# CGLemon/Sayuri

Measured on AMD Instinct MI355X. Metric: nn_evals_per_sec, higher is better.
Workload: dtype f16

## Files before the change

### include/sayuri_hip.h

```cpp
#ifndef SAYURI_HIP_H
#define SAYURI_HIP_H

#include <stddef.h>
#include <stdint.h>

#ifdef __cplusplus
extern "C" {
#endif

typedef struct sayuri_hip_ctx sayuri_hip_ctx;

enum {
    SAYURI_ACT_IDENTITY = 0, SAYURI_ACT_RELU = 1, SAYURI_ACT_ELU = 2, SAYURI_ACT_SELU = 3,
    SAYURI_ACT_GELU = 4, SAYURI_ACT_MISH = 5, SAYURI_ACT_SWISH = 6, SAYURI_ACT_HARDSWISH = 7
};

enum {
    SAYURI_BLOCK_RESIDUAL = 1, SAYURI_BLOCK_BOTTLENECK = 2, SAYURI_BLOCK_NESTED_BOTTLENECK = 3,
    SAYURI_BLOCK_MIXER = 4
};

typedef struct {
    int32_t type;
    int32_t apply_se;
// ... 39 lines not shown
sayuri_hip_ctx* sayuri_hip_create(int device, const sayuri_hip_netdesc* desc, int max_batch,
                                  int board, int use_fp16);

enum { SAYURI_HIP_LATENCY = 1 };
sayuri_hip_ctx* sayuri_hip_create_ex(int device, const sayuri_hip_netdesc* desc, int max_batch,
                                     int board, int use_fp16, unsigned flags);

int sayuri_hip_load_tensor(sayuri_hip_ctx* ctx, int layer_id, int kind, const float* host, size_t n);

int sayuri_hip_forward(sayuri_hip_ctx* ctx, int n, const float* planes, const int* board_sizes,
                       float* prob, float* pass, float* misc, float* own);

int sayuri_hip_upload(sayuri_hip_ctx* ctx, int n, const float* planes, const int* board_sizes);
int sayuri_hip_run(sayuri_hip_ctx* ctx);
int sayuri_hip_sync(sayuri_hip_ctx* ctx);
int sayuri_hip_download(sayuri_hip_ctx* ctx, float* prob, float* pass, float* misc, float* own);

int sayuri_hip_submit(sayuri_hip_ctx* ctx, int n, const float* planes, const int* board_sizes, float* prob,
                      float* pass, float* misc, float* own, int* ticket);
int sayuri_hip_forward_packed(sayuri_hip_ctx* ctx, int n, const unsigned* records, int binary_planes, const int* board_sizes,
                              float* prob, float* pass, float* misc, float* own);
int sayuri_hip_submit_packed(sayuri_hip_ctx* ctx, int n, const unsigned* records, int binary_planes, const int* board_sizes,
                             float* prob, float* pass, float* misc, float* own, int* ticket);
int sayuri_hip_wait(sayuri_hip_ctx* ctx, int ticket);
int sayuri_hip_query(sayuri_hip_ctx* ctx, int ticket);

int sayuri_hip_time_runs(sayuri_hip_ctx* ctx, int iters, float* total_ms);

typedef struct {
    char name[48];
    int32_t launches;
    float total_ms;
    double flops;
    double bytes;
} sayuri_hip_kernel_stat;
int sayuri_hip_profile_run(sayuri_hip_ctx* ctx, sayuri_hip_kernel_stat* rows, int cap);

int sayuri_hip_mark_kernel(sayuri_hip_ctx* ctx, const char* name);
int sayuri_hip_timed_stat(sayuri_hip_ctx* ctx, sayuri_hip_kernel_stat* row);

void* sayuri_hip_host_alloc(size_t bytes);
void sayuri_hip_host_free(void* p);

size_t sayuri_hip_device_bytes(const sayuri_hip_ctx* ctx);

int sayuri_hip_last_chains(const sayuri_hip_ctx* ctx);

int sayuri_hip_tower_state(const sayuri_hip_ctx* ctx);

int sayuri_hip_latency_state(const sayuri_hip_ctx* ctx);

void sayuri_hip_destroy(sayuri_hip_ctx* ctx);

const char* sayuri_hip_last_error(void);

int sayuri_hip_test_conv(int device, int use_fp16, int n, const int* board_sizes, int max_board,
                         int cin, int cout, int k, int depthwise, int act, int post_residual,
                         const float* x, const float* w, const float* bias, const float* res,
                         float* y);
int sayuri_hip_test_conv_split(int device, int n, const int* board_sizes, int max_board, int cin, int cout, int act,
                               const float* x, const float* w, const float* bias, const float* res, float* y,
                               int channel_tiles, int strips);
int sayuri_hip_test_last_conv_kind(void);
int sayuri_hip_test_se_unit(int device, int use_fp16, int n, const int* board_sizes, int max_board, int channels,
                            int se_size, int act, const float* x, const float* res, const float* w1, const float* b1,
                            const float* w2, const float* b2, float* y, float* gate);
int sayuri_hip_test_head_tail(int device, int use_fp16, int n, const int* board_sizes, int max_board, int policy_channels,
                              int value_channels, int prob_channels, int pass_outs, int misc_outs, int act,
                              const float* pconv, const float* vconv, const float* const* weights12, float* prob,
                              float* pass, float* misc, float* own);

int sayuri_hip_test_conv_se(int device, int n, const int* board_sizes, int max_board, int channels, int se_size, int act,
                            int via_tower, const float* x, const float* w, const float* bias, const float* res, const float* w1,
                            const float* b1, const float* w2, const float* b2, float* y);
int sayuri_hip_test_conv_sx(int device, int n, const int* board_sizes, int max_board, int channels, int se_size, int act,
                            const float* x, const float* w, const float* bias, const float* res, const float* w1,
                            const float* b1, const float* w2, const float* b2, float* y);
int sayuri_hip_test_last_sx_kts(void);
int sayuri_hip_test_head_board(int device, int n, const int* board_sizes, int max_board, int channels, int policy_channels,
                               int value_channels, int prob_channels, int pass_outs, int misc_outs, int act, const float* trunk,
                               const float* p_w, const float* p_b, const float* v_w, const float* v_b,
                               const float* const* weights12, float* prob, float* pass, float* misc, float* own);

#ifdef __cplusplus
}
#endif
#endif
```

### sayuri_amd/_lib.py

```python
from __future__ import annotations

import ctypes
import os

from . import _build

c_float_p = ctypes.POINTER(ctypes.c_float)
c_int_p = ctypes.POINTER(ctypes.c_int)


class KernelStat(ctypes.Structure):
    _fields_ = [("name", ctypes.c_char * 48), ("launches", ctypes.c_int32), ("total_ms", ctypes.c_float),
                ("flops", ctypes.c_double), ("bytes", ctypes.c_double)]


HIP_SYMBOLS = [
    "sayuri_hip_device_count", "sayuri_hip_create", "sayuri_hip_create_ex", "sayuri_hip_latency_state", "sayuri_hip_test_conv_split", "sayuri_hip_load_tensor", "sayuri_hip_forward",
    "sayuri_hip_submit", "sayuri_hip_wait", "sayuri_hip_query", "sayuri_hip_upload", "sayuri_hip_run", "sayuri_hip_sync", "sayuri_hip_download", "sayuri_hip_time_runs",
    "sayuri_hip_forward_packed", "sayuri_hip_submit_packed", "sayuri_hip_profile_run", "sayuri_hip_mark_kernel", "sayuri_hip_timed_stat", "sayuri_hip_host_alloc", "sayuri_hip_host_free", "sayuri_hip_device_bytes", "sayuri_hip_last_chains", "sayuri_hip_tower_state",
    "sayuri_hip_destroy", "sayuri_hip_last_error", "sayuri_hip_test_conv", "sayuri_hip_test_last_conv_kind",
    "sayuri_hip_test_se_unit", "sayuri_hip_test_head_tail", "sayuri_hip_test_conv_se", "sayuri_hip_test_head_board",
    "sayuri_hip_test_conv_sx", "sayuri_hip_test_last_sx_kts",
]

_hip = None
_host = None


def _require(path: str) -> str:
    if not os.path.exists(path):
        raise RuntimeError(
            f"native library {path} is missing: run `python -c 'import __graft_entry__ as g; g.build()'` "
            "(there is no CPU fallback for the MI355X forward pipe)")
    return path


def hip() -> ctypes.CDLL:
    global _hip
    if _hip is None:
        path = _build.HIP_SO
        fake = os.environ.get("SAYURI_FAKE_HIP_LIB")
        if fake:
            import sys
            print(f"[sayuri_amd] SAYURI_FAKE_HIP_LIB is set: the device side is the test stand-in {fake}, NOT the MI355X engine",
                  file=sys.stderr)
            path = fake
        lib = ctypes.CDLL(_require(path), mode=ctypes.RTLD_GLOBAL)
        lib.sayuri_hip_last_error.restype = ctypes.c_char_p
        lib.sayuri_hip_device_count.restype = ctypes.c_int
        lib.sayuri_hip_upload.argtypes = [ctypes.c_void_p, ctypes.c_int, c_float_p, c_int_p]
        lib.sayuri_hip_run.argtypes = [ctypes.c_void_p]
        lib.sayuri_hip_sync.argtypes = [ctypes.c_void_p]
        lib.sayuri_hip_download.argtypes = [ctypes.c_void_p, c_float_p, c_float_p, c_float_p, c_float_p]
        lib.sayuri_hip_forward.argtypes = [ctypes.c_void_p, ctypes.c_int, c_float_p, c_int_p, c_float_p,
                                           c_float_p, c_float_p, c_float_p]
        lib.sayuri_hip_time_runs.argtypes = [ctypes.c_void_p, ctypes.c_int, c_float_p]
        lib.sayuri_hip_profile_run.argtypes = [ctypes.c_void_p, ctypes.POINTER(KernelStat), ctypes.c_int]
        lib.sayuri_hip_mark_kernel.argtypes = [ctypes.c_void_p, ctypes.c_char_p]
        lib.sayuri_hip_timed_stat.argtypes = [ctypes.c_void_p, ctypes.POINTER(KernelStat)]
        lib.sayuri_hip_device_bytes.restype = ctypes.c_size_t
        lib.sayuri_hip_device_bytes.argtypes = [ctypes.c_void_p]
        lib.sayuri_hip_last_chains.restype = ctypes.c_int
        lib.sayuri_hip_last_chains.argtypes = [ctypes.c_void_p]
        lib.sayuri_hip_tower_state.restype = ctypes.c_int
        lib.sayuri_hip_tower_state.argtypes = [ctypes.c_void_p]
        if hasattr(lib, "sayuri_hip_latency_state"):
            lib.sayuri_hip_latency_state.restype = ctypes.c_int
            lib.sayuri_hip_latency_state.argtypes = [ctypes.c_void_p]
        if hasattr(lib, "sayuri_hip_create_ex"):
            lib.sayuri_hip_create_ex.restype = ctypes.c_void_p
            lib.sayuri_hip_create_ex.argtypes = [ctypes.c_int, ctypes.c_void_p, ctypes.c_int, ctypes.c_int, ctypes.c_int, ctypes.c_uint]
        if hasattr(lib, "sayuri_hip_test_conv_split"):
            lib.sayuri_hip_test_conv_split.argtypes = [ctypes.c_int, ctypes.c_int, c_int_p, ctypes.c_int, ctypes.c_int, ctypes.c_int,
                                                       ctypes.c_int, c_float_p, c_float_p, c_float_p, c_float_p, c_float_p,
                                                       ctypes.c_int, ctypes.c_int]
        if not fake:
            lib.sayuri_hip_test_conv.argtypes = [ctypes.c_int, ctypes.c_int, ctypes.c_int, c_int_p, ctypes.c_int,
                                                 ctypes.c_int, ctypes.c_int, ctypes.c_int, ctypes.c_int, ctypes.c_int,
                                                 ctypes.c_int, c_float_p, c_float_p, c_float_p, c_float_p, c_float_p]
        _hip = lib
    return _hip


def host() -> ctypes.CDLL:
    global _host
    if _host is None:
        hip()
        lib = ctypes.CDLL(_require(_build.HOST_SO))
        lib.sayuri_host_last_error.restype = ctypes.c_char_p
        lib.sayuri_weights_load.restype = ctypes.c_void_p
        lib.sayuri_weights_load.argtypes = [ctypes.c_char_p]
        lib.sayuri_weights_free.argtypes = [ctypes.c_void_p]
        lib.sayuri_weights_info.argtypes = [ctypes.c_void_p, c_int_p]
        lib.sayuri_weights_block_info.argtypes = [ctypes.c_void_p, ctypes.c_int, c_int_p]
        lib.sayuri_weights_tensor.restype = ctypes.c_long
        lib.sayuri_weights_tensor.argtypes = [ctypes.c_void_p, ctypes.c_char_p, c_float_p, ctypes.c_long]
        lib.sayuri_pipe_create.restype = ctypes.c_void_p
        lib.sayuri_pipe_create.argtypes = [ctypes.c_char_p, ctypes.c_int, ctypes.c_int, ctypes.c_int, ctypes.c_int,
                                           ctypes.c_int]
        lib.sayuri_pipe_create_ex.restype = ctypes.c_void_p
        lib.sayuri_pipe_create_ex.argtypes = [ctypes.c_char_p, ctypes.c_int, ctypes.c_int, ctypes.c_int, ctypes.c_int,
                                              ctypes.c_int, ctypes.c_uint]
        lib.sayuri_pipe_destroy.argtypes = [ctypes.c_void_p]
        lib.sayuri_pipe_num_workers.argtypes = [ctypes.c_void_p]
        lib.sayuri_pipe_ctx.restype = ctypes.c_void_p
# ... 12 lines not shown
```

### sayuri_amd/csrc/hip/engine_graph.h

```cpp
#pragma once
#include "engine_plan.h"

namespace sayuri {

class EngineBase {
public:
    virtual ~EngineBase() {}
    virtual int load_tensor(int layer, int kind, const float* host, size_t n) = 0;
    virtual int upload(int n, const float* planes, const int* board_sizes, const unsigned* packed = nullptr, int binary = 0) = 0;
    virtual int run() = 0;
    virtual int sync() = 0;
    virtual int download(float* prob, float* pass, float* misc, float* own) = 0;
    virtual int time_runs(int iters, float* ms) = 0;
    virtual int profile_run(sayuri_hip_kernel_stat* rows, int cap) = 0;
    virtual int submit(int n, const float* planes, const int* bsz, float* prob, float* pass, float* misc, float* own,
                       int* ticket, const unsigned* packed = nullptr, int binary = 0) = 0;
    virtual int wait(int ticket) = 0;
    virtual int query(int ticket) = 0;
    virtual int mark_kernel(const char* name) = 0;
    virtual int timed_stat(sayuri_hip_kernel_stat* row) = 0;
    virtual size_t device_bytes() const = 0;
    virtual int last_chains() const = 0;
    virtual int tower_state() const = 0;
    virtual int latency_state() const = 0;
// ... 1082 lines not shown
    void rows_reset() {
        for (int i = 0; i < kNumBufs; ++i) rows_stride_[i] = 0;
    }
    int rows_use(const Fwd& f, const ConvParams& p, const char* layer) {
        const void* use[3] = {p.in, p.out, p.res};
        for (int u = 0; u < 3 && flags_.dbg_recycle_input < 2; ++u)
            for (int i = 0; i < kNumBufs; ++i) {
                if (!use[u] || f.io.bufs[i] != use[u]) continue;
                const int stride = u ? p.cout_s : p.cin_s;
                if (rows_stride_[i] && rows_stride_[i] != stride)
                    return fail(std::string("activation buffer ") + std::to_string(i) + " is used with row stride " + std::to_string(stride) + " by " +
                                layer + " and with " + std::to_string(rows_stride_[i]) + " by " + (rows_first_[i] ? rows_first_[i] : "?") +
                                " inside one persistent run / chained forward: the rows of different tiles would overlap");
                rows_stride_[i] = stride;
                rows_first_[i] = layer;
            }
        return 0;
    }

    const ConvLayerDev& cv(int id) const { return convs_.at(id); }
    const FcLayerDev& fc(int id) const { return fcs_.at(id); }

    int forward(int t, float* zc_pass = nullptr, float* zc_misc = nullptr) {
        const int G = chains_for_batch();
        last_chains_ = G;
        rows_reset();
        IoSlot& io = io_[t];
        Fwd f{t, io, compute_[t]};
        f.ntiles = plan().ntiles;
        f.ns = geom_.n;
        f.px = geom_.total;
        f.pass = zc_pass ? zc_pass : io.pass;
        f.misc = zc_misc ? zc_misc : io.misc;
        if (sx_kts_) {
            int nse = 0;
            for (const auto& b : blocks_) nse += b.apply_se ? 1 : 0;
            if (io.sx_epoch > 0xfff00000u) {
                HIP_OK(hipMemsetAsync(io.sx_xchg, 0, sizeof(unsigned long long) * (size_t)max_batch_ * sx_kts_ * kSxMaxSub * kSxSlots, f.stream));
                io.sx_epoch = 0;
            }
            f.sx_epoch0 = io.sx_epoch;
            io.sx_epoch += (unsigned)nse;
        }
        if (G <= 1) return forward_graph(f);
        if (chain_setup(G)) return -1;
        const BoardTabs* tabs = nullptr;
        if (board_tabs(f, &tabs)) return -1;
        HIP_OK(hipEventRecord(chain_fork_, f.stream));
        const int nt = board_plan_.ntiles;
        for (int g = 0; g < G; ++g) {
            Fwd c = f;
            c.stream = chain_stream_[g];
            c.chained = true;
            c.tile0 = (int)((long)nt * g / G);
            c.ntiles = (int)((long)nt * (g + 1) / G) - c.tile0;
            c.n0 = board_plan_.tile_first[c.tile0];
            c.ns = board_plan_.tile_first[c.tile0 + c.ntiles] - c.n0;
            c.px = geom_.off[c.n0 + c.ns] - geom_.off[c.n0];
            hipError_t e = hipStreamWaitEvent(c.stream, chain_fork_, 0);
            if (flags_.chains_serial && g > 0 && e == hipSuccess) e = hipStreamWaitEvent(c.stream, chain_join_[g - 1], 0);
            if (e == hipSuccess && forward_graph(c)) return -1;
            if (e == hipSuccess) e = hipEventRecord(chain_join_[g], c.stream);
            if (e != hipSuccess) return fail(std::string("chained forward: ") + hipGetErrorString(e));
        }
        for (int g = 0; g < G; ++g) HIP_OK(hipStreamWaitEvent(f.stream, chain_join_[g], 0));
        return 0;
    }

    int pack_input(Fwd& f, T* dst) {
        const int cin = desc_.input_channels, cs = cv(SAYURI_L_INPUT_CONV).cin_s, board = board_;
        const int n0 = f.n0, ns = f.ns;
        const double px = f.px;
        const BatchGeom g = dgeom(f.io);
        const IoSlot& io = f.io;
        if (io.packed_binary > 0) {
            const unsigned* rec = io.packed_src ? io.packed_src : io.packed;
            const int split = io.packed_src ? 1 : kPackSplit;
            const int nbin = io.packed_binary, words = nbin * 12 + 8;
            return timed(f, "pack_input", 0, (double)ns * words * 4 + px * cs * sizeof(T), [&] {
                hipLaunchKernelGGL(pack_bits_kernel<T>, dim3(ns * split), dim3(256), 0, f.stream, rec, words, nbin, dst, g, cin, cs,
                                   io.g_perm, n0, split);
            });
        }
        const int grid = ns * kPackSplit;
        const int chunk = pack_input_chunk(slot_pix_, cs, (int)sizeof(T));
        const size_t lds = (size_t)chunk * (cs * sizeof(T) + 16);
        const size_t flat_lds = pack_input_flat_lds(slot_pix_, cs, (int)sizeof(T));
        const bool flat = flat_lds <= 64 * 1024 && (size_t)cin * board * board < 65536;
        return timed(f, "pack_input", 0, px * cin * 4 + px * cs * sizeof(T), [&] {
            if (flat)
                hipLaunchKernelGGL(pack_input_flat_kernel<T>, dim3(ns), dim3(kPackFlatThreads), flat_lds, f.stream,
                                   (const float*)io.planes, dst, g, cin, cs, board, io.g_perm, n0);
            else
                hipLaunchKernelGGL(pack_input_kernel<T>, dim3(grid), dim3(kPackThreads), lds, f.stream,
                                   (const float*)io.planes, dst, g, cin, cs, board, io.g_perm, chunk, n0);
        });
    }

    int forward_graph(Fwd& f) {
        const auto& d = desc_;
        const int C = d.residual_channels, csC = round_up(C, 32), act = d.default_act;
        T* const* buf = f.io.bufs;

        int x = f.take();
        const int in = f.take();
        if (pack_input(f, buf[in])) return -1;
        if (conv(f, "conv3x3_input", cv(SAYURI_L_INPUT_CONV), buf[in], buf[x], nullptr, act)) return -1;
        if (flags_.dbg_recycle_input) f.give(in);

        for (int b = 0; b < d.residual_blocks; ++b) {
            const auto& bd = blocks_[b];
            const bool se = bd.apply_se != 0;
            const int last_act = se ? (int)kIdentity : act;
            const int y = f.take();
            int skip = x;
            bool se_done = false;
            if (bd.type == SAYURI_BLOCK_RESIDUAL) {
                const int t0 = f.take();
                if (conv(f, "conv3x3_tower", cv(SAYURI_L_BLOCK(b, SAYURI_S_CONV1)), buf[x], buf[t0], nullptr, act)) return -1;
                int fused = 1;
                if (se) {
                    fused = conv_se(f, cv(SAYURI_L_BLOCK(b, SAYURI_S_CONV2)), fc(SAYURI_L_BLOCK(b, SAYURI_S_SQUEEZE)),
                                    fc(SAYURI_L_BLOCK(b, SAYURI_S_EXCITE)), buf[t0], buf[y], buf[x], C, act);
                    if (fused == 1)
                        fused = conv_sx(f, cv(SAYURI_L_BLOCK(b, SAYURI_S_CONV2)), fc(SAYURI_L_BLOCK(b, SAYURI_S_SQUEEZE)),
                                        fc(SAYURI_L_BLOCK(b, SAYURI_S_EXCITE)), buf[t0], buf[y], buf[x], C, act);
                    if (fused < 0) return -1;
                    se_done = fused == 0;
                }
                if (fused == 1 &&
                    conv(f, "conv3x3_tower", cv(SAYURI_L_BLOCK(b, SAYURI_S_CONV2)), buf[t0], buf[y], se ? nullptr : buf[x], last_act))
                    return -1;
                f.give(t0);
            } else if (bd.type == SAYURI_BLOCK_BOTTLENECK) {
                const int t0 = f.take(), t1 = f.take();
                if (conv(f, "conv1x1_tower", cv(SAYURI_L_BLOCK(b, SAYURI_S_PRE_BTL)), buf[x], buf[t0], nullptr, act)) return -1;
                if (conv(f, "conv3x3_tower", cv(SAYURI_L_BLOCK(b, SAYURI_S_CONV1)), buf[t0], buf[t1], nullptr, act)) return -1;
                if (conv(f, "conv3x3_tower", cv(SAYURI_L_BLOCK(b, SAYURI_S_CONV2)), buf[t1], buf[t0], nullptr, act)) return -1;
                if (conv(f, "conv1x1_tower", cv(SAYURI_L_BLOCK(b, SAYURI_S_POST_BTL)), buf[t0], buf[y], se ? nullptr : buf[x], last_act)) return -1;
                f.give(t0); f.give(t1);
            } else if (bd.type == SAYURI_BLOCK_NESTED_BOTTLENECK) {
                const int r1 = f.take(), t0 = f.take(), t1 = f.take();
                if (conv(f, "conv1x1_tower", cv(SAYURI_L_BLOCK(b, SAYURI_S_PRE_BTL)), buf[x], buf[r1], nullptr, act)) return -1;
                if (conv(f, "conv3x3_tower", cv(SAYURI_L_BLOCK(b, SAYURI_S_CONV1)), buf[r1], buf[t0], nullptr, act)) return -1;
                if (conv(f, "conv3x3_tower", cv(SAYURI_L_BLOCK(b, SAYURI_S_CONV2)), buf[t0], buf[t1], buf[r1], act)) return -1;
                if (conv(f, "conv3x3_tower", cv(SAYURI_L_BLOCK(b, SAYURI_S_CONV3)), buf[t1], buf[t0], nullptr, act)) return -1;
                if (conv(f, "conv3x3_tower", cv(SAYURI_L_BLOCK(b, SAYURI_S_CONV4)), buf[t0], buf[r1], buf[t1], act)) return -1;
                if (conv(f, "conv1x1_tower", cv(SAYURI_L_BLOCK(b, SAYURI_S_POST_BTL)), buf[r1], buf[y], se ? nullptr : buf[x], last_act)) return -1;
                f.give(r1); f.give(t0); f.give(t1);
            } else {
                const int s2 = f.take(), t1 = f.take();
                if (depthwise(f, "depthwise", cv(SAYURI_L_BLOCK(b, SAYURI_S_DW_CONV)), buf[x], buf[s2], buf[x], act)) return -1;
                if (conv(f, "conv1x1_tower", cv(SAYURI_L_BLOCK(b, SAYURI_S_CONV1)), buf[s2], buf[t1], nullptr, act)) return -1;
                if (conv(f, "conv1x1_tower", cv(SAYURI_L_BLOCK(b, SAYURI_S_CONV2)), buf[t1], buf[y], se ? nullptr : buf[s2], last_act)) return -1;
                f.give(t1);
                f.give(x);
                x = s2;
                skip = s2;
            }
            if (se && !se_done) {
                if (se_unit(f, fc(SAYURI_L_BLOCK(b, SAYURI_S_SQUEEZE)), fc(SAYURI_L_BLOCK(b, SAYURI_S_EXCITE)), buf[y], buf[skip], C, csC,
                            act, f.n0, f.ns))
                    return -1;
            }
            f.give(x);
            x = y;
        }
        return heads(f, x);
    }

    int heads(Fwd& f, int x) {
        const auto& d = desc_;
        const int C = d.residual_channels, csC = round_up(C, 32), act = d.default_act;
        const int Cp = d.policy_head_channels, Cv = d.value_head_channels;
        T* const* buf = f.io.bufs;
        const BatchGeom g = dgeom(f.io);
        const ConvLayerDev &pw = cv(SAYURI_L_PROB_CONV), &ow = cv(SAYURI_L_V_OWNERSHIP);
        const HeadWeights hw{fc(SAYURI_L_P_INTER_FC).dev(), fc(SAYURI_L_PASS_FC).dev(), fc(SAYURI_L_V_INTER_FC).dev(), fc(SAYURI_L_V_MISC).dev(),
                             pw.w32, pw.bias, ow.w32, ow.bias};
// ... 194 lines not shown
```

### sayuri_amd/csrc/hip/engine_plan.h

```cpp
#pragma once
namespace sayuri {

static thread_local std::string g_err;
static std::atomic<unsigned> g_host_free_gen{0};
static thread_local int g_test_conv_kind = 0;
static int fail(const std::string& m) { g_err = m; return -1; }

#define HIP_OK(expr)                                                                      \
    do {                                                                                  \
        hipError_t e_ = (expr);                                                           \
        if (e_ != hipSuccess) {                                                           \
            g_err = std::string(#expr) + ": " + hipGetErrorString(e_);                    \
            return -1;                                                                    \
        }                                                                                 \
    } while (0)

static inline int round_up(int v, int m) { return (v + m - 1) / m * m; }
constexpr size_t kMaxLds = 160 * 1024;
constexpr int kNumCU = 256;

template <typename T> struct ConvKernelTable {
    typedef void (*Fn)(const ConvParams);
    struct Entry { int wmt, wnt; Fn fn; size_t (*lds)(int); int npos_cap; };
    static std::vector<Entry>& entries() {
// ... 487 lines not shown
    img2->assign((size_t)kts * w2_bytes, 0);
    for (int kt = 0; kt < kts; ++kt) {
        for (int bs = 2; bs <= board; ++bs) {
            const float sc = ((float)bs - 14.f) / 10.f;
            f16* d = img1->data() + ((size_t)kt * (board - 1) + (bs - 2)) * (w1_bytes / 2);
            for (int r = 0; r < 256; ++r) {
                const int c = kt * 128 + (r & 127);
                if (c >= C) continue;
                for (int o = 0; o < se; ++o) {
                    const float* w = sq_w + (size_t)o * 3 * C;
                    d[(size_t)r * se + o] = (f16)(r < 128 ? w[c] + sc * w[C + c] : w[2 * C + c]);
                }
            }
        }
        unsigned char* base = img2->data() + (size_t)kt * w2_bytes;
        f16* h = (f16*)base;
        float* bias = (float*)(base + (size_t)se * 256 * 2);
        for (int o = 0; o < 256; ++o) {
            const int c = kt * 128 + (o & 127);
            if (c >= C) continue;
            const int row = o < 128 ? c : C + c;
            for (int i = 0; i < se; ++i) h[((size_t)(i >> 2) * 256 + o) * 4 + (i & 3)] = (f16)ex_w[(size_t)row * se + i];
            bias[o] = ex_b[row];
        }
        std::copy(sq_b, sq_b + se, bias + 256);
    }
    *w1_bytes_out = w1_bytes;
    *w2_bytes_out = w2_bytes;
    return true;
}

struct HeadImages {
    std::vector<f16> img, img2;
    std::vector<float> bias;
    int PT = 0, VT = 0;
};
static HeadFn make_head_images(int C, int Cp, int Cv, int prob_ch, int board, const float* p_w, const float* p_b, const float* v_w,
                               const float* v_b, const float* prob_w, const float* own_w, HeadImages* out) {
    if (board * board > kHeadPix || prob_ch > 8) return nullptr;
    const int PT = round_up(Cp, 16), rows = round_up(PT + Cv, 32), VT = rows - PT, cs = round_up(C, 32), nch = cs / 32;
    HeadFn fn = nullptr;
    for (const auto& e : kHeadEntries)
        if (e.rt * 16 == rows && head_board_fits(rows, nch, e.depth)) { fn = e.fn; break; }
    if (!fn) return nullptr;
    out->img2.assign((size_t)(rows / 32) * 4 * 16 * 8, (f16)0.f);
    for (int t = 0; t < rows / 32; ++t)
        for (int kg = 0; kg < 4; ++kg)
            for (int e = 0; e < 8; ++e) {
                const int ch = 32 * t + (e < 4 ? 4 * kg + e : 16 + 4 * kg + (e - 4));
                for (int k = 0; k < prob_ch; ++k)
                    if (ch < Cp) out->img2[(((size_t)t * 4 + kg) * 16 + k) * 8 + e] = (f16)prob_w[(size_t)k * Cp + ch];
                if (ch >= PT && ch - PT < Cv) out->img2[(((size_t)t * 4 + kg) * 16 + prob_ch) * 8 + e] = (f16)own_w[ch - PT];
            }
    out->img.assign((size_t)nch * 4 * rows * 8, (f16)0.f);
    out->bias.assign(rows, 0.f);
    for (int half = 0; half < 2; ++half) {
        const float* w = half ? v_w : p_w;
        const float* b = half ? v_b : p_b;
        const int cout = half ? Cv : Cp, r0 = half ? PT : 0;
        for (int ko = 0; ko < cout; ++ko) {
            out->bias[r0 + ko] = b[ko];
            for (int c = 0; c < C; ++c)
                out->img[(((size_t)(c / 32) * 4 + (c % 32) / 8) * rows + r0 + ko) * 8 + c % 8] = (f16)w[(size_t)ko * C + c];
        }
    }
    out->PT = PT;
    out->VT = VT;
    return fn;
}

struct HeadWeights {
    FcDev p_inter, pass_fc, v_inter, v_misc;
    const float *prob_w, *prob_b, *own_w, *own_b;
};
static HeadParams head_params(const HeadWeights& w, int Cp, int Cv, int prob_ch, int act, int board, float* prob, float* pass, float* misc,
                              float* own, const int* perm) {
    HeadParams h{};
    h.p_inter = w.p_inter; h.pass_fc = w.pass_fc; h.v_inter = w.v_inter; h.v_misc = w.v_misc;
    h.prob_w = w.prob_w; h.prob_b = w.prob_b; h.own_w = w.own_w; h.own_b = w.own_b;
    h.Cp = Cp; h.cs_p = round_up(Cp, 32); h.Cv = Cv; h.cs_v = round_up(Cv, 32); h.prob_ch = prob_ch; h.act = act; h.board = board;
    h.prob = prob; h.pass = pass; h.misc = misc; h.own = own; h.perm = perm;
    return h;
}
template <typename T, typename Run>
static int se_unit_launches(hipStream_t s, const BatchGeom& g, double px, T* x, const T* res, float* separt, float* gate, const FcDev& sq,
                            const FcDev& ex, int C, int cs, int act, int n0, int ns, Run&& run) {
    constexpr int EPP = ElemTraits<T>::kPieceElems;
    if (cs / EPP > 256) return fail("SE unit: more than 256*8 channels is not supported");
    const double fc = (double)sq.in * sq.out + (double)ex.in * ex.out;
    if (run("se_pool", 2.0 * px * C, sizeof(T) * px * C,
            [&] { hipLaunchKernelGGL(se_pool_kernel<T>, dim3(ns * kSeSplit), dim3(256), 0, s, (const T*)x, separt, g, cs, n0); }))
        return -1;
    const size_t smem = sizeof(float) * (3 * C + sq.out + kSeFcThreads);
    if (run("se_fc", 2.0 * ns * fc, 4.0 * ns * fc, [&] {
            hipLaunchKernelGGL(se_fc_kernel, dim3(ns), dim3(kSeFcThreads), smem, s, (const float*)separt, gate, g, C, cs, sq, ex, act, n0);
        }))
        return -1;
    const dim3 grid((g.slot_pix * (cs / EPP) + 256 * kScaleUnroll - 1) / (256 * kScaleUnroll), ns);
    return run("se_scale", 3.0 * px * C, sizeof(T) * px * C * 3,
               [&] { hipLaunchKernelGGL(se_scale_kernel<T>, grid, dim3(256), 0, s, (const T*)x, res, x, (const float*)gate, g, C, cs, act, n0); });
}

}
extern "C" const unsigned char sayuri_tower_hsaco[];
extern "C" const unsigned long long sayuri_tower_hsaco_size;
namespace sayuri {
static int load_tower_module(hipModule_t* mod, hipFunction_t fn[2]) {
    if (sayuri_tower_hsaco_size == 0) return fail("this build carries no persistent tower kernel: tower_seam.py rejected the compiler's assembly at build time");
    HIP_OK(hipModuleLoadData(mod, sayuri_tower_hsaco));
    HIP_OK(hipModuleGetFunction(&fn[0], *mod, "_ZN6sayuri17conv_tower_kernelILi4EEEvPKNS_10TowerLayerE"));
    HIP_OK(hipModuleGetFunction(&fn[1], *mod, "_ZN6sayuri17conv_tower_kernelILi2EEEvPKNS_10TowerLayerE"));
    return 0;
}

}
```

### sayuri_amd/csrc/hip/engine_taps.h

```cpp
#pragma once
#include "engine_graph.h"

namespace sayuri {

struct TestGeom {
    HostGeom hg;
    int slot = 0;
    int* d_off = nullptr;
    int* d_bsz = nullptr;
    BatchGeom g{};
};

class TestArena {
public:
    ~TestArena() { for (void* p : ptrs_) (void)hipFree(p); }
    void* alloc(size_t bytes) {
        void* p = nullptr;
        if (hipMalloc(&p, std::max<size_t>(bytes, 256)) != hipSuccess) return nullptr;
        (void)hipMemset(p, 0, std::max<size_t>(bytes, 256));
        ptrs_.push_back(p);
        return p;
    }
    template <typename U> U* upload(const std::vector<U>& h) {
        U* d = (U*)alloc(h.size() * sizeof(U));
// ... 339 lines not shown
                             const float* b2, float* y) {
    typedef f16 T;
    constexpr unsigned kEpoch = 0x5e17u;
    g_test_sx_kts = 0;
    HIP_OK(hipSetDevice(device));
    enable_big_lds_glds();
    TestArena A;
    TestGeom tg;
    if (make_test_geom(A, n, board_sizes, max_board, &tg)) return -1;
    const int cs = round_up(C, 32), kts = round_up(C, 128) / 128;
    int wmt, ko_pad;
    conv_tile(cs, true, &wmt, &ko_pad);
    if (cs != kts * 128 || ko_pad != kts * 128) return 1;
    std::vector<f16> img1;
    std::vector<unsigned char> img2;
    int w1_bytes = 0, w2_bytes = 0;
    if (!make_sx_images(C, se, kts, max_board, w1, b1, w2, b2, &img1, &img2, &w1_bytes, &w2_bytes)) return 1;
    const BoardPlan plan = board_plan(tg.hg, ConvOverride{});
    const BoardEntry* be = plan.ok ? sx_board_entry(plan.npos) : nullptr;
    if (!be) return 1;
    for (int i = 0; i < n; ++i)
        if (!sx_board_fused(tg.hg.bsz[i])) return 1;
    const T* dx = A.upload_prefixed(nchw_to_nhwc<T>(tg, x, C, cs));
    const T* dres = res ? A.upload(nchw_to_nhwc<T>(tg, res, C, cs)) : nullptr;
    T* dy = (T*)A.alloc((size_t)n * tg.slot * cs * sizeof(T));
    const T* dw = A.upload(conv_image<T>(w, C, C, 9, ko_pad));
    const float* db = A.upload(padded_bias(bias, C, ko_pad));
    const f16* d1 = A.upload(img1);
    const unsigned char* d2 = A.upload(img2);
    unsigned long long* xchg = (unsigned long long*)A.alloc(sizeof(unsigned long long) * (size_t)plan.ntiles * kts * kSxMaxSub * kSxSlots);
    TestBoardTabs tabs;
    TestHostWord err;
    if (!dx || (res && !dres) || !dy || !dw || !db || !d1 || !d2 || !xchg || !make_board_tabs(A, tg, plan, &tabs) || !err.alloc())
        return fail("test_conv_sx: hipMalloc failed");
    BoardSxParams sp;
    std::memset(&sp, 0, sizeof(sp));
    board_params(sp.b, plan, tabs.src, tabs.pix, tabs.cols, true);
    conv_params(sp.b.c, dx, dw, db, dres, dy, tg.g, cs, cs, ko_pad, 9, act);
    sp.b.c.npos = 0; sp.b.c.num_pix_tiles = plan.ntiles;
    sx_params(sp, d1, d2, w1_bytes, w2_bytes, max_board, se, kts, xchg, kEpoch, err.dev, false);
    HIP_OK(hipMemset(dy, 0xff, (size_t)n * tg.slot * cs * sizeof(T)));
    g_test_conv_kind = kConvBoardSx;
    g_test_sx_kts = kts;
    hipLaunchKernelGGL(conv_board_sx_kernel<2>, dim3(sx_grid(plan.ntiles, kts)), dim3(512), be->lds(plan.npos), 0, sp);
    HIP_OK(hipGetLastError());
    HIP_OK(hipDeviceSynchronize());
    if (*(volatile unsigned*)err.host) return fail("test_conv_sx: a workgroup's wait for its sibling channel tiles ran out");
    return nhwc_to_nchw(tg, dy, C, cs, y);
}

static int test_head_board_impl(int device, int n, const int* board_sizes, int max_board, int C, int Cp, int Cv, int prob_ch,
                                int pass_outs, int misc_outs, int act, const float* trunk, const float* p_w, const float* p_b,
                                const float* v_w, const float* v_b, const float* const* w, float* prob, float* pass, float* misc,
                                float* own) {
    typedef f16 T;
    HIP_OK(hipSetDevice(device));
    enable_big_lds_glds();
    TestArena A;
    TestGeom tg;
    if (make_test_geom(A, n, board_sizes, max_board, &tg)) return -1;
    HeadImages hi;
    const HeadFn fn = make_head_images(C, Cp, Cv, prob_ch, max_board, p_w, p_b, v_w, v_b, w[8], w[10], &hi);
    if (!fn) return 1;
    const int cs = round_up(C, 32);
    const T* dt = A.upload(nchw_to_nhwc<T>(tg, trunk, C, cs));
    const f16* d_img = A.upload(hi.img);
    const f16* d_img2 = A.upload(hi.img2);
    const float* d_bias = A.upload(hi.bias);
    HeadWeights hw;
    TestHeadOut o;
    if (!dt || !d_img || !d_img2 || !d_bias || !upload_head_weights(A, w, Cp, Cv, prob_ch, pass_outs, misc_outs, &hw) ||
        !o.alloc(A, n, prob_ch, pass_outs, misc_outs, max_board * max_board))
        return fail("test_head_board: hipMalloc failed");
    HeadBoardParams hp;
    std::memset(&hp, 0, sizeof(hp));
    hp.h = head_params(hw, Cp, Cv, prob_ch, act, max_board, o.prob, o.pass, o.misc, o.own, nullptr);
    hp.trunk = dt; hp.w = d_img; hp.w2 = d_img2; hp.bias = d_bias; hp.g = tg.g; hp.cs = cs; hp.PT = hi.PT; hp.VT = hi.VT;
    hipLaunchKernelGGL(fn, dim3(n), dim3(512), kMaxLds, 0, hp);
    HIP_OK(hipGetLastError());
    HIP_OK(hipDeviceSynchronize());
    return o.download(prob, pass, misc, own);
}

}

extern "C" int sayuri_hip_test_conv_se(int device, int n, const int* board_sizes, int max_board, int channels, int se_size, int act,
                                       int via_tower, const float* x, const float* w, const float* bias, const float* res,
                                       const float* w1, const float* b1, const float* w2, const float* b2, float* y) {
    if (!board_sizes || !x || !w || !w1 || !b1 || !w2 || !b2 || !y || n <= 0) return fail("test_conv_se: bad argument");
    return test_conv_se_impl(device, n, board_sizes, max_board, channels, se_size, act, via_tower, x, w, bias, res, w1, b1, w2, b2, y);
}

extern "C" int sayuri_hip_test_conv_sx(int device, int n, const int* board_sizes, int max_board, int channels, int se_size, int act,
                                       const float* x, const float* w, const float* bias, const float* res, const float* w1,
                                       const float* b1, const float* w2, const float* b2, float* y) {
    if (!board_sizes || !x || !w || !w1 || !b1 || !w2 || !b2 || !y || n <= 0) return fail("test_conv_sx: bad argument");
    return test_conv_sx_impl(device, n, board_sizes, max_board, channels, se_size, act, x, w, bias, res, w1, b1, w2, b2, y);
}

extern "C" int sayuri_hip_test_last_sx_kts(void) { return sayuri::g_test_sx_kts; }

extern "C" int sayuri_hip_test_head_board(int device, int n, const int* board_sizes, int max_board, int channels, int policy_channels,
                                          int value_channels, int prob_channels, int pass_outs, int misc_outs, int act, const float* trunk,
                                          const float* p_w, const float* p_b, const float* v_w, const float* v_b,
                                          const float* const* weights12, float* prob, float* pass, float* misc, float* own) {
    if (!board_sizes || !trunk || !p_w || !p_b || !v_w || !v_b || !weights12 || !prob || !pass || !misc || !own || n <= 0)
        return fail("test_head_board: bad argument");
    return test_head_board_impl(device, n, board_sizes, max_board, channels, policy_channels, value_channels, prob_channels, pass_outs,
                                misc_outs, act, trunk, p_w, p_b, v_w, v_b, weights12, prob, pass, misc, own);
}

extern "C" int sayuri_hip_test_se_unit(int device, int use_fp16, int n, const int* board_sizes, int max_board, int channels, int se_size,
                                       int act, const float* x, const float* res, const float* w1, const float* b1, const float* w2,
                                       const float* b2, float* y, float* gate) {
    if (!board_sizes || !x || !w1 || !b1 || !w2 || !b2 || !y || n <= 0) return fail("test_se_unit: bad argument");
    if (use_fp16) return test_se_unit_impl<f16>(device, n, board_sizes, max_board, channels, se_size, act, x, res, w1, b1, w2, b2, y, gate);
    return test_se_unit_impl<float>(device, n, board_sizes, max_board, channels, se_size, act, x, res, w1, b1, w2, b2, y, gate);
}

extern "C" int sayuri_hip_test_head_tail(int device, int use_fp16, int n, const int* board_sizes, int max_board, int policy_channels,
                                         int value_channels, int prob_channels, int pass_outs, int misc_outs, int act, const float* pconv,
                                         const float* vconv, const float* const* weights12, float* prob, float* pass, float* misc,
                                         float* own) {
    if (!board_sizes || !pconv || !vconv || !weights12 || !prob || !pass || !misc || !own || n <= 0) return fail("test_head_tail: bad argument");
    if (use_fp16)
        return test_head_tail_impl<f16>(device, n, board_sizes, max_board, policy_channels, value_channels, prob_channels, pass_outs,
                                        misc_outs, act, pconv, vconv, weights12, prob, pass, misc, own);
    return test_head_tail_impl<float>(device, n, board_sizes, max_board, policy_channels, value_channels, prob_channels, pass_outs,
                                      misc_outs, act, pconv, vconv, weights12, prob, pass, misc, own);
}

extern "C" int sayuri_hip_test_conv_split(int device, int n, const int* board_sizes, int max_board, int cin, int cout, int act, const float* x,
                                          const float* w, const float* bias, const float* res, float* y, int channel_tiles, int strips) {
    if (!board_sizes || !x || !w || !y || n <= 0) return fail("test_conv_split: bad argument");
    return test_conv_split_impl(device, n, board_sizes, max_board, cin, cout, act, x, w, bias, res, y, channel_tiles, strips);
}

extern "C" int sayuri_hip_test_last_conv_kind(void) { return sayuri::g_test_conv_kind; }

extern "C" int sayuri_hip_test_conv(int device, int use_fp16, int n, const int* board_sizes, int max_board, int cin,
                                    int cout, int k, int depthwise, int act, int post_residual, const float* x,
                                    const float* w, const float* bias, const float* res, float* y) {
    if (!board_sizes || !x || !w || !y || n <= 0) return fail("test_conv: bad argument");
    if (use_fp16)
        return test_conv_impl<f16>(device, n, board_sizes, max_board, cin, cout, k, depthwise, act, post_residual, x, w,
                                   bias, res, y);
    return test_conv_impl<float>(device, n, board_sizes, max_board, cin, cout, k, depthwise, act, post_residual, x, w,
                                 bias, res, y);
}
```

### sayuri_amd/csrc/hip/small_ops.h

```cpp
#pragma once
#include <algorithm>

#include "common.h"

namespace sayuri {

constexpr int kPackThreads = 128;
constexpr int kPackSplit = 4;
template <typename T>
__global__ __launch_bounds__(kPackThreads) void pack_input_kernel(const float* __restrict__ planes, T* __restrict__ out,
                                                                  BatchGeom g, int cin, int cs, int board, const int* __restrict__ perm,
                                                                  int chunk, int n0 = 0) {
    constexpr int EPP = ElemTraits<T>::kPieceElems;
    extern __shared__ __attribute__((aligned(16))) unsigned char pk_smem[];
    const int n = n0 + blockIdx.x / kPackSplit, part = blockIdx.x % kPackSplit, tid = threadIdx.x;
    const int bs = g.bsz[n], npix = bs * bs, ppr = cs / EPP, stride = cs * (int)sizeof(T) + 16;
    const int per = (npix + kPackSplit - 1) / kPackSplit, pbeg = part * per, pend = min(npix, pbeg + per);
    const size_t B2 = (size_t)board * board;
    const float* src = planes + (size_t)(perm ? perm[n] : n) * cin * B2;
    T* dst = out + (size_t)n * g.slot_pix * cs;
    for (int p0 = pbeg; p0 < pend; p0 += chunk) {
        const int np = min(chunk, pend - p0);
        if (p0 != pbeg) __syncthreads();
        for (int q = tid; q < np; q += kPackThreads) {
            const int pp = p0 + q, y = pp / bs, x = pp - y * bs;
            const float* s0 = src + y * board + x;
            for (int pb = 0; pb < ppr; pb += 6) {
                float f[6 * EPP];
#pragma unroll
                for (int k = 0; k < 6 * EPP; ++k) {
                    const int c = pb * EPP + k;
                    f[k] = c < cin ? s0[(size_t)c * B2] : 0.f;
                }
#pragma unroll
                for (int j = 0; j < 6; ++j) {
                    if (pb + j < ppr) {
                        T v[EPP];
#pragma unroll
                        for (int e = 0; e < EPP; ++e) v[e] = from_float<T>(f[j * EPP + e]);
                        *(uint4*)(pk_smem + (size_t)q * stride + (pb + j) * 16) = *(uint4*)v;
                    }
                }
            }
        }
        __syncthreads();
        for (int it = tid; it < np * ppr; it += kPackThreads) {
            const int q = it / ppr, piece = it - q * ppr;
            *(uint4*)(dst + ((size_t)p0 * ppr + it) * EPP) = *(const uint4*)(pk_smem + (size_t)q * stride + piece * 16);
        }
    }
}
constexpr int kPackFlatThreads = 512;
constexpr int kPackFlatLoads = 32;
template <typename T>
__global__ __launch_bounds__(kPackFlatThreads) void pack_input_flat_kernel(const float* __restrict__ planes, T* __restrict__ out,
                                                                            BatchGeom g, int cin, int cs, int board,
                                                                            const int* __restrict__ perm, int n0 = 0) {
    constexpr int EPP = ElemTraits<T>::kPieceElems;
    extern __shared__ __attribute__((aligned(16))) unsigned char pk_smem[];
    const int n = n0 + blockIdx.x, tid = threadIdx.x;
    const int bs = g.bsz[n], npix = bs * bs, ppr = cs / EPP, stride = cs * (int)sizeof(T) + 16;
    const int B2 = board * board, total = cin * B2;
    const float* src = planes + (size_t)(perm ? perm[n] : n) * total;
    T* dst = out + (size_t)n * g.slot_pix * cs;
    const float r_b2 = 1.0f / (float)B2, r_b = 1.0f / (float)board;
    for (int base = 0; base < total; base += kPackFlatThreads * kPackFlatLoads) {
        float f[kPackFlatLoads];
#pragma unroll
        for (int k = 0; k < kPackFlatLoads; ++k) {
            const int e = base + k * kPackFlatThreads + tid;
            f[k] = e < total ? src[e] : 0.f;
        }
#pragma unroll
        for (int k = 0; k < kPackFlatLoads; ++k) {
            const int e = base + k * kPackFlatThreads + tid;
            const int c = (int)(((float)e + 0.5f) * r_b2), r = e - c * B2;
            const int y = (int)(((float)r + 0.5f) * r_b), x = r - y * board;
            if (e < total && y < bs && x < bs) *(T*)(pk_smem + (size_t)(y * bs + x) * stride + c * (int)sizeof(T)) = from_float<T>(f[k]);
        }
    }
    __syncthreads();
    for (int it = tid; it < npix * ppr; it += kPackFlatThreads) {
        const int q = it / ppr, piece = it - q * ppr;
        T v[EPP];
        *(uint4*)v = *(const uint4*)(pk_smem + (size_t)q * stride + piece * 16);
#pragma unroll
        for (int e = 0; e < EPP; ++e)
            if (piece * EPP + e >= cin) v[e] = from_float<T>(0.f);
        *(uint4*)(dst + (size_t)it * EPP) = *(uint4*)v;
    }
}
static inline size_t pack_input_flat_lds(int slot_pix, int cs, int elem) { return (size_t)slot_pix * (cs * elem + 16); }

static inline int pack_input_chunk(int slot_pix, int cs, int elem) {
    return std::min((slot_pix + kPackSplit - 1) / kPackSplit, (64 * 1024) / (cs * elem + 16));
}

__global__ __launch_bounds__(256) void geom_stage_kernel(const int* __restrict__ stage, int max_batch, int n, int* __restrict__ off,
                                                         int* __restrict__ bsz, int* __restrict__ perm) {
    for (int i = threadIdx.x; i <= n; i += blockDim.x) off[i] = stage[i];
    for (int i = threadIdx.x; i < n; i += blockDim.x) {
        bsz[i] = stage[max_batch + 1 + i];
        perm[i] = stage[2 * max_batch + 1 + i];
    }
}

template <typename T>
__global__ __launch_bounds__(256) void pack_bits_kernel(const unsigned* __restrict__ records, int rec_words, int nbin,
                                                        T* __restrict__ out, BatchGeom g, int cin, int cs,
                                                        const int* __restrict__ perm, int n0 = 0, int split = kPackSplit) {
    constexpr int EPP = ElemTraits<T>::kPieceElems;
    __shared__ unsigned rec[40 * 13 + 8];
    const int n = n0 + blockIdx.x / split, part = blockIdx.x % split, tid = threadIdx.x;
    const int bs = g.bsz[n], npix = bs * bs, ppr = cs / EPP;
    const int per = (npix + split - 1) / split, pbeg = part * per, pend = min(npix, pbeg + per);
    const unsigned* src = records + (size_t)(perm ? perm[n] : n) * rec_words;
    for (int i = tid; i < rec_words; i += 256) rec[i < nbin * 12 ? (i / 12) * 13 + i % 12 : nbin * 13 + (i - nbin * 12)] = src[i];
    __syncthreads();
    T* dst = out + (size_t)n * g.slot_pix * cs;
    for (int it = pbeg * ppr + tid; it < pend * ppr; it += 256) {
        const int pp = it / ppr, piece = it - pp * ppr;
        const int word = pp >> 5, sh = pp & 31;
        T v[EPP];
#pragma unroll
        for (int e = 0; e < EPP; ++e) {
            const int c = piece * EPP + e;
            float f = 0.f;
            if (c < nbin) f = (float)((rec[c * 13 + word] >> sh) & 1u);
            else if (c < cin) f = __uint_as_float(rec[nbin * 13 + (c - nbin)]);
            v[e] = from_float<T>(f);
        }
        *(uint4*)(dst + (size_t)it * EPP) = *(uint4*)v;
    }
}

struct FcDev {
    const float* wt;
    const float* b;
    int in, out;
};

__device__ __forceinline__ void block_fc(const FcDev fc, const float* x, float* y, int act, int tid, int nt) {
    for (int o = tid; o < fc.out; o += nt) {
        float s0 = 0.f, s1 = 0.f;
        const float* w = fc.wt + o;
        int i = 0;
        for (; i + 8 <= fc.in; i += 8) {
            float wv[8];
#pragma unroll
            for (int u = 0; u < 8; ++u) wv[u] = w[(size_t)(i + u) * fc.out];
#pragma unroll
            for (int u = 0; u < 8; u += 2) { s0 += x[i + u] * wv[u]; s1 += x[i + u + 1] * wv[u + 1]; }
        }
        for (; i < fc.in; ++i) s0 += x[i] * w[(size_t)i * fc.out];
        y[o] = activate(fc.b[o] + (s0 + s1), act);
    }
}

template <typename T>
__device__ __forceinline__ void block_pool(const T* __restrict__ x, int npix, int C, int cs, int bs,
                                           bool value_head, float* pool, float* scratch, int tid, int nt) {
    const int cl_n = cs < nt ? cs : nt;
    const int parts = nt / cl_n;
    const int cl = tid % cl_n, part = tid / cl_n;
    for (int c0 = 0; c0 < cs; c0 += cl_n) {
        const int c = c0 + cl;
        float sum = 0.f, mx = -5000.f;
        if (part < parts && c < cs) {
#pragma unroll 8
            for (int p = part; p < npix; p += parts) {
                const float v = to_float(x[(size_t)p * cs + c]);
                sum += v;
                mx = fmaxf(mx, v);
            }
        }
// ... 287 lines not shown
```

Measured before the change: 74270.

## Split flat input-pack kernel by board rows with vectorized float4 loads

The flat input-packing kernel now launches four blocks per sample, each handling a band of board rows, instead of one block per sample. Global reads use aligned float4 loads with a scalar edge fallback, and LDS is staged channel-major with a padded stride to reduce bank conflicts. The transposed pixel-major write is assembled from per-channel LDS reads. This targets a serialized, low-occupancy pre-tower pack step, at the cost of more complex indexing and more scattered LDS reads in the output phase. A test entry point for the pack routine is added.

```diff
diff --git a/include/sayuri_hip.h b/include/sayuri_hip.h
--- a/include/sayuri_hip.h
+++ b/include/sayuri_hip.h
@@ -145,6 +145,9 @@
                                const float* p_w, const float* p_b, const float* v_w, const float* v_b,
                                const float* const* weights12, float* prob, float* pass, float* misc, float* own);
 
+int sayuri_hip_test_pack_input(int device, int use_fp16, int n, const int* board_sizes, int max_board, int cin, const float* planes,
+                               const int* perm, void* out);
+
 #ifdef __cplusplus
 }
 #endif
diff --git a/sayuri_amd/_lib.py b/sayuri_amd/_lib.py
--- a/sayuri_amd/_lib.py
+++ b/sayuri_amd/_lib.py
@@ -20,7 +20,7 @@
     "sayuri_hip_forward_packed", "sayuri_hip_submit_packed", "sayuri_hip_profile_run", "sayuri_hip_mark_kernel", "sayuri_hip_timed_stat", "sayuri_hip_host_alloc", "sayuri_hip_host_free", "sayuri_hip_device_bytes", "sayuri_hip_last_chains", "sayuri_hip_tower_state",
     "sayuri_hip_destroy", "sayuri_hip_last_error", "sayuri_hip_test_conv", "sayuri_hip_test_last_conv_kind",
     "sayuri_hip_test_se_unit", "sayuri_hip_test_head_tail", "sayuri_hip_test_conv_se", "sayuri_hip_test_head_board",
-    "sayuri_hip_test_conv_sx", "sayuri_hip_test_last_sx_kts",
+    "sayuri_hip_test_conv_sx", "sayuri_hip_test_last_sx_kts", "sayuri_hip_test_pack_input",
 ]
 
 _hip = None
diff --git a/sayuri_amd/csrc/hip/engine_graph.h b/sayuri_amd/csrc/hip/engine_graph.h
--- a/sayuri_amd/csrc/hip/engine_graph.h
+++ b/sayuri_amd/csrc/hip/engine_graph.h
@@ -1188,19 +1188,8 @@
                                    io.g_perm, n0, split);
             });
         }
-        const int grid = ns * kPackSplit;
-        const int chunk = pack_input_chunk(slot_pix_, cs, (int)sizeof(T));
-        const size_t lds = (size_t)chunk * (cs * sizeof(T) + 16);
-        const size_t flat_lds = pack_input_flat_lds(slot_pix_, cs, (int)sizeof(T));
-        const bool flat = flat_lds <= 64 * 1024 && (size_t)cin * board * board < 65536;
-        return timed(f, "pack_input", 0, px * cin * 4 + px * cs * sizeof(T), [&] {
-            if (flat)
-                hipLaunchKernelGGL(pack_input_flat_kernel<T>, dim3(ns), dim3(kPackFlatThreads), flat_lds, f.stream,
-                                   (const float*)io.planes, dst, g, cin, cs, board, io.g_perm, n0);
-            else
-                hipLaunchKernelGGL(pack_input_kernel<T>, dim3(grid), dim3(kPackThreads), lds, f.stream,
-                                   (const float*)io.planes, dst, g, cin, cs, board, io.g_perm, chunk, n0);
-        });
+        return timed(f, "pack_input", 0, px * cin * 4 + px * cs * sizeof(T),
+                     [&] { pack_input_launch<T>(f.stream, (const float*)io.planes, dst, g, cin, cs, board, io.g_perm, n0, ns); });
     }
 
     int forward_graph(Fwd& f) {
diff --git a/sayuri_amd/csrc/hip/engine_plan.h b/sayuri_amd/csrc/hip/engine_plan.h
--- a/sayuri_amd/csrc/hip/engine_plan.h
+++ b/sayuri_amd/csrc/hip/engine_plan.h
@@ -593,6 +593,20 @@
     h.prob = prob; h.pass = pass; h.misc = misc; h.own = own; h.perm = perm;
     return h;
 }
+template <typename T>
+static void pack_input_launch(hipStream_t s, const float* planes, T* dst, const BatchGeom& g, int cin, int cs, int board, const int* perm,
+                              int n0, int ns) {
+    const size_t flat_lds = pack_input_flat_lds(board, cin, (int)sizeof(T));
+    if (flat_lds <= 64 * 1024 && (size_t)cin * board * board < 65536) {
+        hipLaunchKernelGGL(pack_input_flat_kernel<T>, dim3(ns * kPackFlatSplit), dim3(kPackFlatThreads), flat_lds, s, planes, dst, g, cin, cs,
+                           board, perm, n0);
+        return;
+    }
+    const int chunk = pack_input_chunk(g.slot_pix, cs, (int)sizeof(T));
+    const size_t lds = (size_t)chunk * (cs * sizeof(T) + 16);
+    hipLaunchKernelGGL(pack_input_kernel<T>, dim3(ns * kPackSplit), dim3(kPackThreads), lds, s, planes, dst, g, cin, cs, board, perm, chunk,
+                       n0);
+}
 template <typename T, typename Run>
 static int se_unit_launches(hipStream_t s, const BatchGeom& g, double px, T* x, const T* res, float* separt, float* gate, const FcDev& sq,
                             const FcDev& ex, int C, int cs, int act, int n0, int ns, Run&& run) {
diff --git a/sayuri_amd/csrc/hip/engine_taps.h b/sayuri_amd/csrc/hip/engine_taps.h
--- a/sayuri_amd/csrc/hip/engine_taps.h
+++ b/sayuri_amd/csrc/hip/engine_taps.h
@@ -445,6 +445,28 @@
     return o.download(prob, pass, misc, own);
 }
 
+template <typename T>
+static int test_pack_input_impl(int device, int n, const int* board_sizes, int max_board, int cin, const float* planes, const int* perm,
+                                void* out) {
+    HIP_OK(hipSetDevice(device));
+    TestArena A;
+    TestGeom tg;
+    if (make_test_geom(A, n, board_sizes, max_board, &tg)) return -1;
+    const int cs = round_up(cin, 32);
+    const size_t n_out = (size_t)n * tg.slot * cs;
+    const float* dp = A.upload(std::vector<float>(planes, planes + (size_t)n * cin * tg.slot));
+    const int* dperm = perm ? A.upload(std::vector<int>(perm, perm + n)) : nullptr;
+    T* dy = (T*)A.alloc(n_out * sizeof(T));
+    if (!dp || !dy || (perm && !dperm)) return fail("test_pack_input: hipMalloc failed");
+    HIP_OK(hipMemset(dy, 0xff, n_out * sizeof(T)));
+    HIP_OK(hipDeviceSynchronize());
+    pack_input_launch<T>(0, dp, dy, tg.g, cin, cs, max_board, dperm, 0, n);
+    HIP_OK(hipGetLastError());
+    HIP_OK(hipDeviceSynchronize());
+    HIP_OK(hipMemcpy(out, dy, n_out * sizeof(T), hipMemcpyDeviceToHost));
+    return 0;
+}
+
 }
 
 extern "C" int sayuri_hip_test_conv_se(int device, int n, const int* board_sizes, int max_board, int channels, int se_size, int act,
@@ -459,6 +481,13 @@
                                        const float* b1, const float* w2, const float* b2, float* y) {
     if (!board_sizes || !x || !w || !w1 || !b1 || !w2 || !b2 || !y || n <= 0) return fail("test_conv_sx: bad argument");
     return test_conv_sx_impl(device, n, board_sizes, max_board, channels, se_size, act, x, w, bias, res, w1, b1, w2, b2, y);
+}
+
+extern "C" int sayuri_hip_test_pack_input(int device, int use_fp16, int n, const int* board_sizes, int max_board, int cin,
+                                          const float* planes, const int* perm, void* out) {
+    if (!board_sizes || !planes || !out || n <= 0 || cin <= 0) return fail("test_pack_input: bad argument");
+    if (use_fp16) return test_pack_input_impl<f16>(device, n, board_sizes, max_board, cin, planes, perm, out);
+    return test_pack_input_impl<float>(device, n, board_sizes, max_board, cin, planes, perm, out);
 }
 
 extern "C" int sayuri_hip_test_last_sx_kts(void) { return sayuri::g_test_sx_kts; }
diff --git a/sayuri_amd/csrc/hip/small_ops.h b/sayuri_amd/csrc/hip/small_ops.h
--- a/sayuri_amd/csrc/hip/small_ops.h
+++ b/sayuri_amd/csrc/hip/small_ops.h
@@ -50,47 +50,76 @@
         }
     }
 }
-constexpr int kPackFlatThreads = 512;
-constexpr int kPackFlatLoads = 32;
+constexpr int kPackFlatThreads = 256;
+constexpr int kPackFlatSplit = 4;
+constexpr int kPackFlatLoads = 8;
+__host__ __device__ static inline int pack_flat_row0(int board, int part) { return part * board / kPackFlatSplit; }
+__host__ __device__ static inline int pack_flat_stride(int board) {
+    const int rows = (board + kPackFlatSplit - 1) / kPackFlatSplit;
+    return ((rows * board + 15) & ~15) + 1;
+}
 template <typename T>
 __global__ __launch_bounds__(kPackFlatThreads) void pack_input_flat_kernel(const float* __restrict__ planes, T* __restrict__ out,
                                                                             BatchGeom g, int cin, int cs, int board,
                                                                             const int* __restrict__ perm, int n0 = 0) {
     constexpr int EPP = ElemTraits<T>::kPieceElems;
     extern __shared__ __attribute__((aligned(16))) unsigned char pk_smem[];
-    const int n = n0 + blockIdx.x, tid = threadIdx.x;
-    const int bs = g.bsz[n], npix = bs * bs, ppr = cs / EPP, stride = cs * (int)sizeof(T) + 16;
-    const int B2 = board * board, total = cin * B2;
-    const float* src = planes + (size_t)(perm ? perm[n] : n) * total;
-    T* dst = out + (size_t)n * g.slot_pix * cs;
-    const float r_b2 = 1.0f / (float)B2, r_b = 1.0f / (float)board;
-    for (int base = 0; base < total; base += kPackFlatThreads * kPackFlatLoads) {
-        float f[kPackFlatLoads];
+    T* img = (T*)pk_smem;
+    const int n = n0 + blockIdx.x / kPackFlatSplit, part = blockIdx.x % kPackFlatSplit, tid = threadIdx.x;
+    const int bs = g.bsz[n], ppr = cs / EPP, PS = pack_flat_stride(board);
+    const int y0 = pack_flat_row0(board, part), y1 = pack_flat_row0(board, part + 1);
+    const int B2 = board * board, total = cin * B2, L = (y1 - y0) * board;
+    const int Q = (L + 6) >> 2;
+    const float* src = planes + (size_t)(perm ? perm[n] : n) * total + y0 * board;
+    const float* end = planes + (size_t)g.n_samples * total;
+    const int rows = min(y1, bs) - min(y0, bs), npix = rows * bs;
+    T* dst = out + ((size_t)n * g.slot_pix + (size_t)min(y0, bs) * bs) * cs;
+    const float r_q = 1.0f / (float)Q, r_b = 1.0f / (float)board;
+    for (int base = 0; base < cin * Q && rows > 0; base += kPackFlatThreads * kPackFlatLoads) {
+        float f[kPackFlatLoads][4];
+        int c[kPackFlatLoads], r0[kPackFlatLoads];
 #pragma unroll
         for (int k = 0; k < kPackFlatLoads; ++k) {
-            const int e = base + k * kPackFlatThreads + tid;
-            f[k] = e < total ? src[e] : 0.f;
+            const int item = base + k * kPackFlatThreads + tid;
+            c[k] = (int)(((float)item + 0.5f) * r_q);
+            const int j = item - c[k] * Q;
+            const float* run = src + (size_t)c[k] * B2;
+            const int a = (int)(((size_t)run >> 2) & 3);
+            r0[k] = 4 * j - a;
+            const float* q = run + r0[k];
+            if (c[k] >= cin || r0[k] >= L) {
+                r0[k] = L;
+            } else if (q >= planes && q + 4 <= end) {
+                *(float4*)f[k] = *(const float4*)q;
+            } else {
+#pragma unroll
+                for (int e = 0; e < 4; ++e) f[k][e] = (r0[k] + e >= 0 && r0[k] + e < L) ? q[e] : 0.f;
+            }
         }
 #pragma unroll
         for (int k = 0; k < kPackFlatLoads; ++k) {
-            const int e = base + k * kPackFlatThreads + tid;
-            const int c = (int)(((float)e + 0.5f) * r_b2), r = e - c * B2;
-            const int y = (int)(((float)r + 0.5f) * r_b), x = r - y * board;
-            if (e < total && y < bs && x < bs) *(T*)(pk_smem + (size_t)(y * bs + x) * stride + c * (int)sizeof(T)) = from_float<T>(f[k]);
+#pragma unroll
+            for (int e = 0; e < 4; ++e) {
+                const int r = r0[k] + e;
+                if (r < 0 || r >= L) continue;
+                const int yy = (int)(((float)r + 0.5f) * r_b), x = r - yy * board;
+                if (y0 + yy < bs && x < bs) img[c[k] * PS + yy * bs + x] = from_float<T>(f[k][e]);
+            }
         }
     }
     __syncthreads();
     for (int it = tid; it < npix * ppr; it += kPackFlatThreads) {
-        const int q = it / ppr, piece = it - q * ppr;
+        const int p = it / ppr, piece = it - p * ppr;
         T v[EPP];
-        *(uint4*)v = *(const uint4*)(pk_smem + (size_t)q * stride + piece * 16);
-#pragma unroll
-        for (int e = 0; e < EPP; ++e)
-            if (piece * EPP + e >= cin) v[e] = from_float<T>(0.f);
+#pragma unroll
+        for (int e = 0; e < EPP; ++e) {
+            const int ch = piece * EPP + e;
+            v[e] = ch < cin ? img[ch * PS + p] : from_float<T>(0.f);
+        }
         *(uint4*)(dst + (size_t)it * EPP) = *(uint4*)v;
     }
 }
-static inline size_t pack_input_flat_lds(int slot_pix, int cs, int elem) { return (size_t)slot_pix * (cs * elem + 16); }
+static inline size_t pack_input_flat_lds(int board, int cin, int elem) { return (size_t)cin * pack_flat_stride(board) * elem; }
 
 static inline int pack_input_chunk(int slot_pix, int cs, int elem) {
     return std::min((slot_pix + kPackSplit - 1) / kPackSplit, (64 * 1024) / (cs * elem + 16));
```

Result: no change. 74790, median of 6 (+0.7%).
